# jiangzhengkai/mxdetection

Measured on AMD Instinct MI355X. Metric: images/sec (whole node) Faster R-CNN R50-FPN 3x800x1333, higher is better.
Workload: dtype bf16; 1 GPU; Faster R-CNN ResNet-50-FPN bf16 train step, batch 2/GPU, 3x800x1333 (padded 1344); global_batch=2, parallelism=dp1, frozen=stem+C2, frozen BN folded, optimizer=SGD momentum 0.9 wd 1e-4, launch=hipGraph replay, input=resident, wgrad_side_stream=True, rpn_branch_stream=True, grouped_wgrad=True, filter_prefetch_hints=True, params_trainable=41538304

## Files before the change

include/mxdet.h:

```cpp
#ifndef MXDET_H_
#define MXDET_H_

#include <stddef.h>
#include <stdint.h>

#ifdef __cplusplus
extern "C" {
#endif

#define MXDET_OK 0
#define MXDET_EINVAL (-1)
#define MXDET_ESHAPE (-2)
#define MXDET_EWORKSPACE (-3)
#define MXDET_EHIP (-4)
#define MXDET_ERCCL (-5)

#define MXDET_DTYPE_F32 0
#define MXDET_DTYPE_BF16 1

typedef void* mxdet_stream_t;

const char* mxdet_last_error(void);
const char* mxdet_version(void);

// ... 355 lines not shown
  float eps;
  int32_t relu;
  int32_t accumulate;
} mxdet_gn_desc_t;
size_t mxdet_group_norm_workspace_bytes(const mxdet_gn_desc_t* d, int32_t backward);
int mxdet_group_norm_fwd(const mxdet_gn_desc_t* d, const uint16_t* x, const float* gamma, const float* beta, uint16_t* y,
                         float* mean, float* rstd, void* workspace, size_t workspace_bytes, mxdet_stream_t stream);
int mxdet_group_norm_bwd(const mxdet_gn_desc_t* d, const uint16_t* x, const uint16_t* dy, const uint16_t* y,
                         const float* mean, const float* rstd, const float* gamma, const float* beta, uint16_t* dx,
                         float* dgamma, float* dbeta, void* workspace, size_t workspace_bytes, mxdet_stream_t stream);

int mxdet_stem_conv7x7(const void* image, int32_t dtype, int32_t N, int32_t H, int32_t W,
                       const uint16_t* w, const float* bias, uint16_t* y, mxdet_stream_t stream);
int mxdet_stem_conv7x7_pool(const void* image, int32_t dtype, int32_t N, int32_t H, int32_t W,
                            const uint16_t* w, const float* bias, uint16_t* y, mxdet_stream_t stream);
int mxdet_maxpool3x3s2(const uint16_t* x, int32_t N, int32_t H, int32_t W, int32_t C, uint16_t* y,
                       mxdet_stream_t stream);
int mxdet_subsample2(const uint16_t* x, int32_t N, int32_t H, int32_t W, int32_t C, uint16_t* y,
                     mxdet_stream_t stream);
int mxdet_subsample2_bwd(const uint16_t* dy, int32_t N, int32_t H, int32_t W, int32_t C,
                         int32_t accumulate, uint16_t* dx, mxdet_stream_t stream);
int mxdet_upsample2_bwd(const uint16_t* dfine, int32_t N, int32_t Hf, int32_t Wf, int32_t C,
                        int32_t accumulate, uint16_t* dcoarse, mxdet_stream_t stream);
size_t mxdet_retina_detect_workspace_bytes(const mxdet_pyramid_t* p, int32_t N, int32_t pre_nms_top_n);
int mxdet_retina_detect(const mxdet_pyramid_t* p, int32_t N, const float* im_info, int32_t pre_nms_top_n,
                        float score_thresh, float nms_thresh, int32_t max_per_image, float* dets, int32_t* num_dets,
                        void* workspace, size_t workspace_bytes, mxdet_stream_t stream);
int mxdet_retina_detect_soft(const mxdet_pyramid_t* p, int32_t N, const float* im_info, int32_t pre_nms_top_n,
                             float score_thresh, float nms_thresh, int32_t max_per_image, float* dets,
                             int32_t* num_dets, void* workspace, size_t workspace_bytes, int32_t method, float sigma,
// ... 57 lines not shown
```

include/mxdet_debug.h:

```cpp
#ifndef MXDET_DEBUG_H_
#define MXDET_DEBUG_H_

#include <stdint.h>

#include "mxdet.h"

#ifdef __cplusplus
extern "C" {
#endif

int mxdet_debug_force_conv_cfg(int32_t cfg);
int mxdet_debug_force_wgrad_ksplit(int32_t ksplit);
int mxdet_debug_preprocess_direct(int32_t on);

#define MXDET_TUNE_T64 0
#define MXDET_TUNE_T128 1
#define MXDET_TUNE_PAR64 2
#define MXDET_TUNE_WG_TARGET 3
#define MXDET_TUNE_WG_MINSTEPS 4
#define MXDET_TUNE_WG_MAXSTEPS 5
#define MXDET_TUNE_T3_ENABLE 6
#define MXDET_TUNE_T3_TARGET 7
#define MXDET_TUNE_T3_MINSTEPS 8
#define MXDET_TUNE_T3_NS 9
#define MXDET_TUNE_TAIL 10
#define MXDET_TUNE_WG_NS 11
#define MXDET_TUNE_ROI_TABLE 12
#define MXDET_TUNE_ROI_ROWS 13
#define MXDET_TUNE_STATIC_TAPS 14
#define MXDET_TUNE_T128W 15
#define MXDET_TUNE_T3_MIX 16
#define MXDET_TUNE_SPLITK_TILE 17
#define MXDET_TUNE_T3_PER_ITEM 18
#define MXDET_TUNE_COUNT 19
int mxdet_debug_set_tuning(int32_t which, int64_t value);
int64_t mxdet_debug_get_tuning(int32_t which);


#define MXDET_ROUTE_CONV 1
#define MXDET_ROUTE_WGRAD 2
#define MXDET_ROUTE_CONV_GROUPED 3
#define MXDET_ROUTE_WGRAD_GROUPED 4
#define MXDET_ROUTE_RETINA_LOSS 5
#define MXDET_ROUTE_RETINA_LOSS_IOU 6
#define MXDET_ROUTE_RETINA_LOSS_QUALITY 7
#define MXDET_ROUTE_RETINA_LOSS_DFL 8
#define MXDET_ROUTE_WORDS 16
#define MXDET_ROUTE_MAX 4
int mxdet_debug_route_probe(int32_t on);
int mxdet_debug_route_read(int32_t* records, int32_t max_records);

// ... 9 lines not shown
```

mxdetection_amd/_lib.py:

```python
import ctypes as C
import os

_HERE = os.path.dirname(os.path.abspath(__file__))
LIB_PATH = os.environ.get("MXDET_LIB") or os.path.join(_HERE, "libmxdet_hip.so")

c_i32, c_i64, c_u32, c_f32, c_sz, c_vp = C.c_int32, C.c_int64, C.c_uint32, C.c_float, C.c_size_t, C.c_void_p


class PyramidT(C.Structure):
    _fields_ = [
        ("num_levels", c_i32), ("A", c_i32),
        ("H", c_i32 * 8), ("W", c_i32 * 8), ("stride", c_i32 * 8),
        ("cls", c_vp * 8), ("reg", c_vp * 8),
        ("cls_sn", c_i64 * 8), ("cls_sy", c_i64 * 8), ("cls_sx", c_i64 * 8), ("cls_sa", c_i64 * 8),
        ("reg_sn", c_i64 * 8), ("reg_sy", c_i64 * 8), ("reg_sx", c_i64 * 8), ("reg_sc", c_i64 * 8),
        ("dtype", c_i32), ("classes", c_i32),
        ("base_anchors", c_vp * 8),
    ]


class FeatPyramidT(C.Structure):
    _fields_ = [
        ("num_levels", c_i32), ("lvl_min", c_i32),
        ("H", c_i32 * 8), ("W", c_i32 * 8),
# ... 187 lines not shown
    "mxdet_deform_im2col": (c_i32, [P(DeformDescT), c_vp, c_vp, c_vp, c_vp]),
    "mxdet_deform_col2im_coord": (c_i32, [P(DeformDescT), c_vp, c_vp, c_vp, c_vp, c_vp]),
    "mxdet_deform_col2im_workspace_bytes": (c_sz, [P(DeformDescT)]),
    "mxdet_deform_col2im": (c_i32, [P(DeformDescT), c_vp, c_vp, c_vp, c_vp, c_sz, c_vp]),
    "mxdet_dpool_fwd": (c_i32, [P(DpoolDescT), c_vp, c_vp, c_i64, c_vp, c_vp, c_vp, c_vp]),
    "mxdet_dpool_bwd_trans": (c_i32, [P(DpoolDescT), c_vp, c_vp, c_i64, c_vp, c_vp, c_vp, c_vp, c_vp, c_vp]),
    "mxdet_dpool_bwd_feat_workspace_bytes": (c_sz, [P(DpoolDescT), c_i64]),
    "mxdet_dpool_bwd_feat": (c_i32, [P(DpoolDescT), c_vp, c_vp, c_i64, c_vp, c_vp, c_vp, c_vp, c_sz, c_vp]),
    "mxdet_group_norm_workspace_bytes": (c_sz, [P(GnDescT), c_i32]),
    "mxdet_group_norm_fwd": (c_i32, [P(GnDescT), c_vp, c_vp, c_vp, c_vp, c_vp, c_vp, c_vp, c_sz, c_vp]),
    "mxdet_group_norm_bwd": (c_i32, [P(GnDescT), c_vp, c_vp, c_vp, c_vp, c_vp, c_vp, c_vp, c_vp, c_vp, c_vp, c_vp, c_sz,
                                     c_vp]),
    "mxdet_debug_group_norm_route": (c_i32, [P(GnDescT)]),
    "mxdet_stem_conv7x7": (c_i32, [c_vp, c_i32, c_i32, c_i32, c_i32, c_vp, c_vp, c_vp, c_vp]),
    "mxdet_stem_conv7x7_pool": (c_i32, [c_vp, c_i32, c_i32, c_i32, c_i32, c_vp, c_vp, c_vp, c_vp]),
    "mxdet_maxpool3x3s2": (c_i32, [c_vp, c_i32, c_i32, c_i32, c_i32, c_vp, c_vp]),
    "mxdet_subsample2": (c_i32, [c_vp, c_i32, c_i32, c_i32, c_i32, c_vp, c_vp]),
    "mxdet_subsample2_bwd": (c_i32, [c_vp, c_i32, c_i32, c_i32, c_i32, c_i32, c_vp, c_vp]),
    "mxdet_upsample2_bwd": (c_i32, [c_vp, c_i32, c_i32, c_i32, c_i32, c_i32, c_vp, c_vp]),
    "mxdet_add_bf16": (c_i32, [c_vp, c_vp, c_i64, c_vp, c_vp]),
    "mxdet_relu_bwd_bf16": (c_i32, [c_vp, c_vp, c_i64, c_vp, c_vp]),
    "mxdet_f32_to_bf16": (c_i32, [c_vp, c_i64, c_vp, c_vp]),
    "mxdet_f32_accum_to_bf16": (c_i32, [c_vp, c_i64, c_i32, c_vp, c_vp]),
    "mxdet_nchw_to_nhwc_bf16": (c_i32, [c_vp, c_i32, c_i32, c_i32, c_i32, c_i32, c_vp, c_vp]),
    "mxdet_nhwc_to_nchw_f32": (c_i32, [c_vp, c_i32, c_i32, c_i32, c_i32, c_vp, c_vp]),
    "mxdet_sgd_momentum_update": (c_i32, [c_vp, c_vp, c_vp, c_vp, c_i64, c_f32, c_f32, c_f32, c_f32, c_vp]),
    "mxdet_sgd_momentum_update_sched": (c_i32, [c_vp, c_vp, c_vp, c_vp, c_i64, c_vp, c_f32, c_f32, c_f32, c_vp]),
    "mxdet_comm_unique_id": (c_i32, [c_vp]),
    "mxdet_comm_create": (c_i32, [c_vp, c_i32, c_i32, P(c_vp)]),
    "mxdet_comm_destroy": (c_i32, [c_vp]),
    "mxdet_allreduce_bucket": (c_i32, [c_vp, c_vp, c_i64, c_vp, P(c_i32)]),
    "mxdet_comm_wait": (c_i32, [c_vp, c_i32, c_vp]),
    "mxdet_comm_broadcast": (c_i32, [c_vp, c_vp, c_sz, c_i32, c_vp]),
    "mxdet_debug_set_tuning": (c_i32, [c_i32, c_i64]),
    "mxdet_debug_get_tuning": (c_i64, [c_i32]),
    "mxdet_debug_route_probe": (c_i32, [c_i32]),
    "mxdet_debug_route_read": (c_i32, [P(c_i32), c_i32]),
}

DEBUG_SYMBOLS = ("mxdet_debug_force_conv_cfg", "mxdet_debug_force_wgrad_ksplit", "mxdet_debug_preprocess_direct",
                 "mxdet_debug_set_tuning", "mxdet_debug_get_tuning", "mxdet_debug_route_probe", "mxdet_debug_route_read",
                 "mxdet_debug_group_norm_route")
TUNING_KEYS = {"T64": 0, "T128": 1, "PAR64": 2, "WG_TARGET": 3, "WG_MINSTEPS": 4, "WG_MAXSTEPS": 5, "T3_ENABLE": 6,
               "T3_TARGET": 7, "T3_MINSTEPS": 8, "T3_NS": 9, "TAIL": 10, "WG_NS": 11, "ROI_TABLE": 12, "ROI_ROWS": 13, "STATIC_TAPS": 14,
               "T128W": 15, "T3_MIX": 16, "SPLITK_TILE": 17, "T3_PER_ITEM": 18}
ROUTE_KINDS = {"CONV": 1, "WGRAD": 2, "CONV_GROUPED": 3, "WGRAD_GROUPED": 4, "RETINA_LOSS": 5, "RETINA_LOSS_IOU": 6,
               "RETINA_LOSS_QUALITY": 7, "RETINA_LOSS_DFL": 8}

IOU_LOSS_KINDS = {"iou": 0, "giou": 1, "diou": 2}
CLS_LOSS_KINDS = {"qfl": 1, "vfl": 2}
CLS_LOSS_KINDS_DFL = {"focal": 0, "qfl": 1, "vfl": 2}
REG_MAX_LIMIT = 31

_lib = None


class MxdetError(RuntimeError):
    pass


# ... 38 lines not shown
```

mxdetection_amd/csrc/capi.hip:

```cpp
#include <stdarg.h>

#include "common.h"

namespace mxdet {

static thread_local char g_err[512] = {0};

void set_error(const char* fmt, ...) {
  va_list ap;
  va_start(ap, fmt);
  vsnprintf(g_err, sizeof(g_err), fmt, ap);
  va_end(ap);
}
void clear_error() { g_err[0] = 0; }

thread_local int g_route_probe = 0;
static thread_local int g_route_n = 0;
static thread_local int32_t g_route[kRouteMax][kRouteWords];
void route_record(const int32_t (&rec)[kRouteWords]) {
  if (g_route_n < kRouteMax) memcpy(g_route[g_route_n], rec, sizeof(rec));
  ++g_route_n;
}

static const long long kTuneDefault[MXDET_TUNE_COUNT] = {400, 1536, 1600, 3072, 64, 128, 1, 1536, 32, 2, 2, 2, 0, 2, 1, 1000000, 1, 0, 192};
static long long g_tune[MXDET_TUNE_COUNT] = {400, 1536, 1600, 3072, 64, 128, 1, 1536, 32, 2, 2, 2, 0, 2, 1, 1000000, 1, 0, 192};
long long tuning(int which) { return g_tune[which]; }

}

extern "C" const char* mxdet_last_error(void) { return mxdet::g_err; }
extern "C" const char* mxdet_version(void) { return "mxdet-hip 0.2 gfx950"; }

extern "C" int mxdet_debug_set_tuning(int32_t which, int64_t value) {
  mxdet::clear_error();
  MXDET_REQUIRE(which >= 0 && which < MXDET_TUNE_COUNT, MXDET_EINVAL, "debug_set_tuning: unknown key %d", which);
  mxdet::g_tune[which] = value < 0 ? mxdet::kTuneDefault[which] : (long long)value;
  return MXDET_OK;
}

extern "C" int64_t mxdet_debug_get_tuning(int32_t which) {
// ... 20 lines not shown
```

mxdetection_amd/csrc/dense_misc.hip:

```cpp
#include "common.h"

namespace mxdet {

typedef __attribute__((ext_vector_type(8))) short s16x8_t;

constexpr int STEM_PW = 264;
constexpr int STEM_PLANE = 7 * STEM_PW;
constexpr int STEM_K = 160;

__global__ void __launch_bounds__(256)
stem_conv_kernel(const void* __restrict__ img, int dtype, int N, int H, int W, int Ho, int Wo,
                 const uint16_t* __restrict__ w, const float* __restrict__ bias,
                 uint16_t* __restrict__ y) {
  constexpr int PATCH_ELEMS = (3 * STEM_PLANE + 8 + 7) & ~7;
  constexpr int MAIN_BYTES = (PATCH_ELEMS + 64 * STEM_K) * 2;
  constexpr int EP_BYTES = 4 * 32 * 68 * 4;
  __shared__ __attribute__((aligned(16))) unsigned char smem_raw[MAIN_BYTES > EP_BYTES ? MAIN_BYTES : EP_BYTES];
  __shared__ int koff[STEM_K];
  uint16_t* patch = (uint16_t*)smem_raw;
  uint16_t* wl = patch + PATCH_ELEMS;
  float* ep = (float*)smem_raw;
  const int tid = threadIdx.x, lane = tid & 63, wid = tid >> 6;
  const int wtiles = ceil_div(Wo, 128);
  int b = blockIdx.x;
// ... 94 lines not shown
constexpr int SP_PW = 296;
constexpr int SP_ROWS = 15;
constexpr int SP_PATCH_BYTES = SP_ROWS * SP_PW * 8;
constexpr int SP_HB_BYTES = 2 * 128 * 64 * 2;
constexpr int SP_LDS = SP_PATCH_BYTES > SP_HB_BYTES ? SP_PATCH_BYTES : SP_HB_BYTES;

template <typename T>
__device__ __forceinline__ float stem_px(const T* p);
template <>
__device__ __forceinline__ float stem_px<float>(const float* p) { return *p; }
template <>
__device__ __forceinline__ float stem_px<uint16_t>(const uint16_t* p) { return bf16_bits_to_f32(*p); }

template <typename T>
__global__ void __launch_bounds__(256, 2)
stem_pool_kernel(const T* __restrict__ img, int N, int H, int W, int Ho, int Wo, int Hp, int Wp,
                 const uint16_t* __restrict__ w, const float* __restrict__ bias, uint16_t* __restrict__ y) {
  __shared__ __attribute__((aligned(16))) unsigned char smem[SP_LDS];
  const int tid = threadIdx.x, lane = tid & 63;
  const int wid = __builtin_amdgcn_readfirstlane(tid >> 6);
  const int wm = wid >> 1, wn = wid & 1;
  const int frow = lane & 15, fq = lane >> 4;
  const int wtiles = ceil_div(Wp, SP_PC), htiles = ceil_div(Hp, 2);
  int b = blockIdx.x;
  const int wt = b % wtiles; b /= wtiles;
  const int ht = b % htiles;
  const int n = b / htiles;
  const int ph0 = 2 * ht, pw0 = wt * SP_PC;
  const int cr0 = 2 * ph0 - 1, cc0 = 2 * pw0 - 1;
  const int ir0 = 2 * cr0 - 3, ic0 = 2 * cc0 - 3;

  {
// ... 128 lines not shown
    if (ph >= Hp || pwg >= Wp) continue;
    const uint4 a = *(const uint4*)(hb + (q * 128 + 2 * pw) * 64 + cg * 8);
    const uint4 c = *(const uint4*)(hb + (q * 128 + 2 * pw + 1) * 64 + cg * 8);
    const uint4 d = *(const uint4*)(hb + (q * 128 + 2 * pw + 2) * 64 + cg * 8);
    auto mx = [](unsigned x, unsigned y2) {
      const unsigned lo = (x & 0xffffu) > (y2 & 0xffffu) ? (x & 0xffffu) : (y2 & 0xffffu);
      const unsigned hi = (x >> 16) > (y2 >> 16) ? (x >> 16) : (y2 >> 16);
      return lo | (hi << 16);
    };
    uint4 o;
    o.x = mx(mx(a.x, c.x), d.x); o.y = mx(mx(a.y, c.y), d.y); o.z = mx(mx(a.z, c.z), d.z); o.w = mx(mx(a.w, c.w), d.w);
    *(uint4*)(y + (((size_t)n * Hp + ph) * Wp + pwg) * 64 + cg * 8) = o;
  }
}


__global__ void maxpool3x3s2_kernel(const uint16_t* __restrict__ x, int N, int H, int W, int C, int Ho,
                                    int Wo, uint16_t* __restrict__ y) {
  const int CG = C >> 3;
  long long idx = (long long)blockIdx.x * blockDim.x + threadIdx.x;
  long long total = (long long)N * Ho * Wo * CG;
  if (idx >= total) return;
  int cg = (int)(idx % CG);
  long long pix = idx / CG;
  int wo = (int)(pix % Wo);
  long long t = pix / Wo;
  int ho = (int)(t % Ho), n = (int)(t / Ho);
  float m[8];
#pragma unroll
  for (int k = 0; k < 8; ++k) m[k] = -3.0e38f;
// ... 216 lines not shown
                     N, H, W, Ho, Wo, w, bias, y);
  return check_launch("stem_conv7x7");
}

extern "C" int mxdet_stem_conv7x7_pool(const void* image, int32_t dtype, int32_t N, int32_t H, int32_t W,
                                       const uint16_t* w, const float* bias, uint16_t* y, mxdet_stream_t stream) {
  clear_error();
  MXDET_REQUIRE(N > 0 && H > 0 && W > 0, MXDET_ESHAPE, "stem_conv7x7_pool: bad shape");
  MXDET_REQUIRE(dtype == MXDET_DTYPE_F32 || dtype == MXDET_DTYPE_BF16, MXDET_EINVAL, "stem_conv7x7_pool: dtype");
  MXDET_REQUIRE(image && w && y, MXDET_EINVAL, "stem_conv7x7_pool: null pointer");
  const int Ho = (H + 6 - 7) / 2 + 1, Wo = (W + 6 - 7) / 2 + 1;
  const int Hp = (Ho + 2 - 3) / 2 + 1, Wp = (Wo + 2 - 3) / 2 + 1;
  const long long nwg = (long long)N * ceil_div(Hp, 2) * ceil_div(Wp, SP_PC);
  MXDET_REQUIRE(nwg < (1ll << 31), MXDET_ESHAPE, "stem_conv7x7_pool: image too large");
  if (dtype == MXDET_DTYPE_F32)
    hipLaunchKernelGGL(stem_pool_kernel<float>, dim3((unsigned)nwg), dim3(256), 0, as_stream(stream), (const float*)image,
                       N, H, W, Ho, Wo, Hp, Wp, w, bias, y);
  else
    hipLaunchKernelGGL(stem_pool_kernel<uint16_t>, dim3((unsigned)nwg), dim3(256), 0, as_stream(stream),
                       (const uint16_t*)image, N, H, W, Ho, Wo, Hp, Wp, w, bias, y);
  return check_launch("stem_conv7x7_pool");
}

extern "C" int mxdet_maxpool3x3s2(const uint16_t* x, int32_t N, int32_t H, int32_t W, int32_t C,
                                  uint16_t* y, mxdet_stream_t stream) {
  clear_error();
  MXDET_REQUIRE(N > 0 && H > 0 && W > 0 && C > 0 && C % 8 == 0, MXDET_ESHAPE, "maxpool3x3s2: bad shape");
  MXDET_REQUIRE(x && y, MXDET_EINVAL, "maxpool3x3s2: null pointer");
  int Ho = (H + 2 - 3) / 2 + 1, Wo = (W + 2 - 3) / 2 + 1;
  long long total = (long long)N * Ho * Wo * (C / 8);
  hipLaunchKernelGGL(maxpool3x3s2_kernel, dim3(blocks_for(total, 256)), dim3(256), 0, as_stream(stream), x,
                     N, H, W, C, Ho, Wo, y);
  return check_launch("maxpool3x3s2");
}

extern "C" int mxdet_subsample2(const uint16_t* x, int32_t N, int32_t H, int32_t W, int32_t C,
// ... 124 lines not shown
```

mxdetection_amd/models/backbones/resnet.py:

```python
import os

import torch

from ...ops import dense
from ..utils.layers import ConvLayer, DeformConvLayer, cached_buf


BITMASKS = os.environ.get("MXDET_TUNE_RELU_BITS", "1") == "1"
CHAIN_FROZEN = os.environ.get("MXDET_TUNE_CHAIN", "1") != "0"
CHAIN3_FROZEN = os.environ.get("MXDET_TUNE_CHAIN", "2") not in ("0", "1")


class Bottleneck:
    def __init__(self, name, cin, planes, stride, downsample, trainable, need_dx, arena, ws, device, gen, dcn=None):
        kw = dict(arena=arena, ws=ws, device=device, gen=gen, trainable=trainable, train_bias=False)
        self.trainable, self.need_dx = trainable, need_dx
        self.conv3 = ConvLayer(name + ".conv3", planes, planes * 4, 1, init_std=0.25 * (2.0 / planes) ** 0.5, **kw)
        self.dcn = dcn is not None
        if self.dcn:
            assert trainable, "deformable convolutions only in trainable stages"
            self.conv2 = DeformConvLayer(name + ".conv2", planes, planes, stride, dcn["groups"], dcn["modulated"],
                                         arena=arena, ws=ws, device=device, gen=gen)
        else:
            self.conv2 = ConvLayer(name + ".conv2", planes, planes, 3, stride, **kw)
# ... 104 lines not shown
        cins = [64, 256, 512, 1024]
        for si in (3, 2, 1, 0):
            planes = 64 << si
            trainable = si > frozen_stages - 1 and si >= 1 if frozen_stages >= 1 else True
            stage = []
            for bi in reversed(range(blocks[si])):
                cin = cins[si] if bi == 0 else planes * 4
                stride = 2 if (bi == 0 and si > 0) else 1
                need_dx = trainable and not (bi == 0 and (si == 0 or si - 1 < frozen_stages))
                stage.insert(0, Bottleneck("layer%d.%d" % (si + 1, bi), cin, planes, stride, bi == 0, trainable,
                                           need_dx, arena, ws, device, gen,
                                           dcn=dcn if si + 2 in dcn_stages else None))
            self.stages[si] = stage
        self.stem_w = (torch.randn((64, 7, 7, 3), generator=gen) * (2.0 / 147) ** 0.5).to(torch.bfloat16).to(device)
        self.stem_b = torch.zeros((64,), dtype=torch.float32, device=device)
        self.bufs = {}
        self.outs = None
        self.front_override = None
        self.eager_parity = 0
        self.front_outs = []

    def layers(self):
        return [l for st in self.stages for b in st for l in b.layers()]

    def plan(self, image_shape):
        N, _, H, W = image_shape
        s = (N, ((H - 1) // 2 + 1 - 1) // 2 + 1, ((W - 1) // 2 + 1 - 1) // 2 + 1, 64)
        shapes = []
        for st in self.stages:
            for b in st:
# ... 2 lines not shown
        return shapes

    def forward(self, image):
        if self.front_override is not None:
            return self.forward_rest(self.front_override)
        return self.forward_rest(self.forward_front(image, self.eager_parity))

    def frozen_front(self):
        n = 0
        for st in self.stages:
            if any(b.trainable for b in st):
                break
            n += 1
        return n

    def forward_front(self, image, parity=0):
        N, _, H, W = image.shape
        H1, W1 = (H - 1) // 2 + 1, (W - 1) // 2 + 1
        dev = self.stem_w.device
        x = dense.stem_conv7x7_pool(image, self.stem_w, self.stem_b,
                                    cached_buf(self.bufs, "pool", (N, (H1 - 1) // 2 + 1, (W1 - 1) // 2 + 1, 64),
                                               torch.bfloat16, dev))
        nf = self.frozen_front()
        if nf > 0:
            self.stages[nf - 1][-1].y_key = "y%d" % parity if parity else "y"
        self.front_outs = []
        for st in self.stages[:nf]:
            x = self._stage_forward(st, x, None)
            self.front_outs.append(x)
        return x

    def _stage_forward(self, st, x, xb):
        ready = False
        for i, b in enumerate(st):
            nb = st[i + 1] if i + 1 < len(st) else None
            ride = (CHAIN3_FROZEN and nb is not None and b.chainable() and nb.chainable() and nb.down is None and
                    nb.conv1.cout == 64 and nb.conv1.stride == 1)
# ... 37 lines not shown
```

mxdetection_amd/models/utils/checkpoint.py:

```python
import torch


class CheckpointMixin:
    def export_params(self):
        out = {"stem.weight": self.backbone.stem_w.float().cpu(), "stem.bias": self.backbone.stem_b.float().cpu()}
        frozen = [l for st in self.backbone.stages for b in st for l in b.layers() if not l.trainable]
        for l in self.layers + frozen:
            out[l.name + ".weight"] = l.w_bf16.float().cpu()
            if l.has_bias:
                out[l.name + ".bias"] = l.bias_f32.float().cpu()
        for l in getattr(self, "norm_layers", ()):
            for name, idx in l.named_params():
                out[name] = self.arena.view(idx, "w").float().cpu()
        return out


    def _named_tensors(self):
        out = [("stem.weight", "frozen", self.backbone.stem_w, None), ("stem.bias", "frozen", self.backbone.stem_b, None)]
        frozen = [l for st in self.backbone.stages for b in st for l in b.layers() if not l.trainable]
        seen = set()
        for l in list(self.layers) + frozen:
            if id(l) in seen:
                continue
            seen.add(id(l))
# ... 71 lines not shown
            by_name[name] = layer
            a = blob.get("arg:" + name)
            if a is None:
                missing.append(name)
                continue
            t.copy_(self._from_mx(a, t, layer).to(t.dtype))
        for i, e in enumerate(self.arena.entries):
            a = blob.get("aux:momentum:" + e[0])
            if a is not None:
                m = self.arena.view(i, "m")
                m.copy_(self._from_mx(a, m, by_name.get(e[0])))
        if strict and missing:
            raise KeyError("checkpoint lacks %d parameters, e.g. %s" % (len(missing), missing[:3]))
        self.arena.refresh_bf16()
        self.refresh_transposed()
        return missing

    def export_grads(self):
        return {e[0]: self.arena.view(i, "g").float().cpu() for i, e in enumerate(self.arena.entries)}

    def num_params(self):
        return sum(e[3] for e in self.arena.entries)
```

mxdetection_amd/models/utils/detector.py:

```python
import contextlib
import os

import torch

from ...utils.hipgraph import GraphEvent
from .checkpoint import CheckpointMixin
from .dp import BucketReducer, make_comm
from .layers import ParamArena, Workspace
from .schedule import CapturedStep, ReplayScratch, ScheduleRecorder, begin_capture, uncovered_ranges


_PROBE_STREAMS = []
_ABL = frozenset(t for t in os.environ.get("MXDET_ABL_SKIP", "").split(",") if t)
Workspace.abl_skip = _ABL


class DetectorBase(CheckpointMixin):
    def _init_base(self, device):
        self.device = device
        self.arena = ParamArena(device)
        self.ws = Workspace(device)
        self.planned = None
        self.dist = None
        self.comm = None
# ... 168 lines not shown
    @contextlib.contextmanager
    def _weights_restored(self):
        snap = (self.arena.w.clone(), self.arena.m.clone())
        yield
        torch.cuda.synchronize()
        self.arena.w.copy_(snap[0])
        self.arena.m.copy_(snap[1])
        self.arena.refresh_bf16()
        self.refresh_transposed()
        del snap
        torch.cuda.synchronize()

    def capture(self, image, gt_boxes, im_info, lr, image_offset=0, warmup=2, gt_masks=None, momentum=0.9, wd=1e-4):
        dev = self.device
        hyper = (float(momentum), float(wd))
        self.static_in = (image.clone(), gt_boxes.clone(), im_info.clone())
        self.static_masks = gt_masks.clone() if gt_masks is not None else None
        self.step_dev = torch.zeros((1,), dtype=torch.int32, device=dev)
        self.lr_dev = torch.full((1,), float(lr), dtype=torch.float32, device=dev)
        self._lr_host = lr

        def eager_step(step):
            self.train_step(*self.static_in, step=step, image_offset=image_offset, lr=lr, gt_masks=self.static_masks,
                            momentum=hyper[0], wd=hyper[1])
        if warmup > 0:
            with self._weights_restored():
                for i in range(warmup):
                    eager_step(i)
        torch.cuda.synchronize()
        cap = CapturedStep()
# ... 178 lines not shown
```

mxdetection_amd/ops/dense.py:

```python
import ctypes as C

import torch

from .. import _lib
from .._lib import ConvDescT, check, ptr, stream_ptr

_DT = {torch.float32: 0, torch.bfloat16: 1}


def mem_range(*tensors):
    spans = [(t.data_ptr(), t.numel() * t.element_size()) for t in tensors]
    bases = {t.untyped_storage().data_ptr() for t in tensors}
    if len(bases) == 1:
        lo = min(p for p, _ in spans)
        hi = max(p + n for p, n in spans)
        if hi - lo <= 2 * sum(n for _, n in set(spans)):
            return (lo, hi - lo)
    return spans[0]


def conv_desc(N, H, W, Cin, Cout, KH, KW, stride, pad, relu=False, res_upsample=False, accumulate=False, prefetch=None,
              relu_bits=None):
    d = ConvDescT()
    if relu_bits is not None:
# ... 224 lines not shown
    check(_lib.load().mxdet_filter_transpose_batched(ptr(table), ndesc, total_tiles, stream_ptr()),
          "filter_transpose_batched")


def stem_conv7x7(image, w, bias=None, out=None):
    lib = _lib.load()
    N, _, H, W = image.shape
    Ho, Wo = (H - 1) // 2 + 1, (W - 1) // 2 + 1
    if out is None:
        out = torch.empty((N, Ho, Wo, 64), dtype=torch.bfloat16, device=image.device)
    check(lib.mxdet_stem_conv7x7(ptr(image), _DT[image.dtype], N, H, W, ptr(w), ptr(bias), ptr(out), stream_ptr()),
          "stem_conv7x7")
    return out


def stem_conv7x7_pool(image, w, bias=None, out=None):
    lib = _lib.load()
    N, _, H, W = image.shape
    Ho, Wo = (H - 1) // 2 + 1, (W - 1) // 2 + 1
    Hp, Wp = (Ho - 1) // 2 + 1, (Wo - 1) // 2 + 1
    if out is None:
        out = torch.empty((N, Hp, Wp, 64), dtype=torch.bfloat16, device=image.device)
    check(lib.mxdet_stem_conv7x7_pool(ptr(image), _DT[image.dtype], N, H, W, ptr(w), ptr(bias), ptr(out), stream_ptr()),
          "stem_conv7x7_pool")
    return out


def maxpool3x3s2(x, out=None):
    lib = _lib.load()
    N, H, W, Cc = x.shape
    Ho, Wo = (H - 1) // 2 + 1, (W - 1) // 2 + 1
    if out is None:
        out = torch.empty((N, Ho, Wo, Cc), dtype=torch.bfloat16, device=x.device)
    check(lib.mxdet_maxpool3x3s2(ptr(x), N, H, W, Cc, ptr(out), stream_ptr()), "maxpool3x3s2")
    return out


# ... 107 lines not shown
```

mxdetection_amd/utils/pretrained.py:

```python
import numpy as np

from .params_io import fold_batchnorm, load_params

_BLOCKS = {50: (3, 4, 6, 3), 101: (3, 4, 23, 3)}


def resnet_v1_names(depth):
    yield "stem", "conv0_weight", "bn0"
    for si, nb in enumerate(_BLOCKS[depth]):
        for bi in range(nb):
            u, ours = "stage%d_unit%d" % (si + 1, bi + 1), "layer%d.%d" % (si + 1, bi)
            for k in (1, 2, 3):
                yield "%s.conv%d" % (ours, k), "%s_conv%d_weight" % (u, k), "%s_bn%d" % (u, k)
            if bi == 0:
                yield ours + ".down", u + "_sc_weight", u + "_sc_bn"


def _get(blob, name):
    for k in ("arg:" + name, "aux:" + name, name):
        if k in blob:
            return np.asarray(blob[k])
    return None


# ... 13 lines not shown
            continue
        wf, bf = fold_batchnorm(w, stats[0], stats[1], stats[2], stats[3], eps=eps, fix_gamma=fix_gamma)
        tw, tb = tensors[ours + ".weight"], tensors[ours + ".bias"]
        src = torch.from_numpy(wf).permute(0, 2, 3, 1).contiguous()
        khwc = getattr(layers[ours + ".weight"], "dcn_khwc", None)
        if khwc is not None and tuple(src.shape[1:]) == tuple(khwc):
            src = src.reshape(tw.shape)
        if tuple(src.shape) != tuple(tw.shape):
            raise ValueError("%s: %s has shape %s, the model expects %s" % (ours, wname, tuple(src.shape), tuple(tw.shape)))
        tw.copy_(src.to(tw.device).to(tw.dtype))
        tb.copy_(torch.from_numpy(bf).to(tb.device).to(tb.dtype))
    if strict and missing:
        raise KeyError("pretrained file lacks %d backbone tensors, e.g. %s" % (len(missing), missing[:3]))
    model.arena.refresh_bf16()
    model.refresh_transposed()
    return missing
```

Measured before the change: 476.3 images/sec.

## Stream stem conv+pool through a row ring buffer with prepacked MFMA filter fragments

Adds a new fused stem 7x7 conv + 3x3 maxpool kernel. Each workgroup walks several pooled row pairs over a column strip, keeping a 16-row image ring in LDS and prefetching the next rows into registers while the MFMAs run, so overlapping input rows are reused instead of reloaded per tile. The stem filter is repacked once into MFMA fragment layout outside the captured graph, and each wave loads it straight into registers. The new route is on by default through a tuning knob. It needs extra state to keep the prepared filter in sync with weight updates, but the stem is frozen here, so this should hold.

```diff
diff --git a/include/mxdet.h b/include/mxdet.h
--- a/include/mxdet.h
+++ b/include/mxdet.h
@@ -393,6 +393,11 @@
                        const uint16_t* w, const float* bias, uint16_t* y, mxdet_stream_t stream);
 int mxdet_stem_conv7x7_pool(const void* image, int32_t dtype, int32_t N, int32_t H, int32_t W,
                             const uint16_t* w, const float* bias, uint16_t* y, mxdet_stream_t stream);
+#define MXDET_STEM_FRAG_BYTES 28672
+int mxdet_stem_filter_prepare(const uint16_t* w, uint16_t* frag, mxdet_stream_t stream);
+int mxdet_stem_conv7x7_pool_prepared(const void* image, int32_t dtype, int32_t N, int32_t H, int32_t W,
+                                     const uint16_t* w, const uint16_t* frag, const float* bias, uint16_t* y,
+                                     mxdet_stream_t stream);
 int mxdet_maxpool3x3s2(const uint16_t* x, int32_t N, int32_t H, int32_t W, int32_t C, uint16_t* y,
                        mxdet_stream_t stream);
 int mxdet_subsample2(const uint16_t* x, int32_t N, int32_t H, int32_t W, int32_t C, uint16_t* y,
diff --git a/include/mxdet_debug.h b/include/mxdet_debug.h
--- a/include/mxdet_debug.h
+++ b/include/mxdet_debug.h
@@ -32,9 +32,11 @@
 #define MXDET_TUNE_T3_MIX 16
 #define MXDET_TUNE_SPLITK_TILE 17
 #define MXDET_TUNE_T3_PER_ITEM 18
-#define MXDET_TUNE_COUNT 19
+#define MXDET_TUNE_STEM_STREAM 19
+#define MXDET_TUNE_COUNT 20
 int mxdet_debug_set_tuning(int32_t which, int64_t value);
 int64_t mxdet_debug_get_tuning(int32_t which);
+int mxdet_debug_stem_stream_geometry(int32_t* strip, int32_t* run_pairs);
 
 
 #define MXDET_ROUTE_CONV 1
diff --git a/mxdetection_amd/_lib.py b/mxdetection_amd/_lib.py
--- a/mxdetection_amd/_lib.py
+++ b/mxdetection_amd/_lib.py
@@ -225,6 +225,9 @@
     "mxdet_debug_group_norm_route": (c_i32, [P(GnDescT)]),
     "mxdet_stem_conv7x7": (c_i32, [c_vp, c_i32, c_i32, c_i32, c_i32, c_vp, c_vp, c_vp, c_vp]),
     "mxdet_stem_conv7x7_pool": (c_i32, [c_vp, c_i32, c_i32, c_i32, c_i32, c_vp, c_vp, c_vp, c_vp]),
+    "mxdet_stem_filter_prepare": (c_i32, [c_vp, c_vp, c_vp]),
+    "mxdet_stem_conv7x7_pool_prepared": (c_i32, [c_vp, c_i32, c_i32, c_i32, c_i32, c_vp, c_vp, c_vp, c_vp, c_vp]),
+    "mxdet_debug_stem_stream_geometry": (c_i32, [P(c_i32), P(c_i32)]),
     "mxdet_maxpool3x3s2": (c_i32, [c_vp, c_i32, c_i32, c_i32, c_i32, c_vp, c_vp]),
     "mxdet_subsample2": (c_i32, [c_vp, c_i32, c_i32, c_i32, c_i32, c_vp, c_vp]),
     "mxdet_subsample2_bwd": (c_i32, [c_vp, c_i32, c_i32, c_i32, c_i32, c_i32, c_vp, c_vp]),
@@ -251,10 +254,10 @@
 
 DEBUG_SYMBOLS = ("mxdet_debug_force_conv_cfg", "mxdet_debug_force_wgrad_ksplit", "mxdet_debug_preprocess_direct",
                  "mxdet_debug_set_tuning", "mxdet_debug_get_tuning", "mxdet_debug_route_probe", "mxdet_debug_route_read",
-                 "mxdet_debug_group_norm_route")
+                 "mxdet_debug_group_norm_route", "mxdet_debug_stem_stream_geometry")
 TUNING_KEYS = {"T64": 0, "T128": 1, "PAR64": 2, "WG_TARGET": 3, "WG_MINSTEPS": 4, "WG_MAXSTEPS": 5, "T3_ENABLE": 6,
                "T3_TARGET": 7, "T3_MINSTEPS": 8, "T3_NS": 9, "TAIL": 10, "WG_NS": 11, "ROI_TABLE": 12, "ROI_ROWS": 13, "STATIC_TAPS": 14,
-               "T128W": 15, "T3_MIX": 16, "SPLITK_TILE": 17, "T3_PER_ITEM": 18}
+               "T128W": 15, "T3_MIX": 16, "SPLITK_TILE": 17, "T3_PER_ITEM": 18, "STEM_STREAM": 19}
 ROUTE_KINDS = {"CONV": 1, "WGRAD": 2, "CONV_GROUPED": 3, "WGRAD_GROUPED": 4, "RETINA_LOSS": 5, "RETINA_LOSS_IOU": 6,
                "RETINA_LOSS_QUALITY": 7, "RETINA_LOSS_DFL": 8}
 
diff --git a/mxdetection_amd/csrc/capi.hip b/mxdetection_amd/csrc/capi.hip
--- a/mxdetection_amd/csrc/capi.hip
+++ b/mxdetection_amd/csrc/capi.hip
@@ -22,8 +22,8 @@
   ++g_route_n;
 }
 
-static const long long kTuneDefault[MXDET_TUNE_COUNT] = {400, 1536, 1600, 3072, 64, 128, 1, 1536, 32, 2, 2, 2, 0, 2, 1, 1000000, 1, 0, 192};
-static long long g_tune[MXDET_TUNE_COUNT] = {400, 1536, 1600, 3072, 64, 128, 1, 1536, 32, 2, 2, 2, 0, 2, 1, 1000000, 1, 0, 192};
+static const long long kTuneDefault[MXDET_TUNE_COUNT] = {400, 1536, 1600, 3072, 64, 128, 1, 1536, 32, 2, 2, 2, 0, 2, 1, 1000000, 1, 0, 192, 1};
+static long long g_tune[MXDET_TUNE_COUNT] = {400, 1536, 1600, 3072, 64, 128, 1, 1536, 32, 2, 2, 2, 0, 2, 1, 1000000, 1, 0, 192, 1};
 long long tuning(int which) { return g_tune[which]; }
 
 }
diff --git a/mxdetection_amd/csrc/dense_misc.hip b/mxdetection_amd/csrc/dense_misc.hip
--- a/mxdetection_amd/csrc/dense_misc.hip
+++ b/mxdetection_amd/csrc/dense_misc.hip
@@ -132,8 +132,8 @@
 
 template <typename T>
 __global__ void __launch_bounds__(256, 2)
-stem_pool_kernel(const T* __restrict__ img, int N, int H, int W, int Ho, int Wo, int Hp, int Wp,
-                 const uint16_t* __restrict__ w, const float* __restrict__ bias, uint16_t* __restrict__ y) {
+stem_pool_oneshot_kernel(const T* __restrict__ img, int N, int H, int W, int Ho, int Wo, int Hp, int Wp,
+                         const uint16_t* __restrict__ w, const float* __restrict__ bias, uint16_t* __restrict__ y) {
   __shared__ __attribute__((aligned(16))) unsigned char smem[SP_LDS];
   const int tid = threadIdx.x, lane = tid & 63;
   const int wid = __builtin_amdgcn_readfirstlane(tid >> 6);
@@ -292,6 +292,223 @@
   }
 }
 
+constexpr int SS_MT = 2;
+constexpr int SS_MG = 1;
+constexpr int SS_R = 2;
+constexpr int SS_COLS = 32 * SS_MT;
+constexpr int SS_PC = SS_MT == 2 ? 28 : 56;
+constexpr int SS_LC = 2 * SS_COLS;
+constexpr int SS_PW = SS_LC + 8;
+constexpr int SS_RPP = 256 / SS_LC;
+constexpr int SS_NPASS = 8 / SS_RPP;
+constexpr int SS_RING_BYTES = 16 * SS_PW * 8;
+constexpr int SS_HB_BYTES = 2 * SS_COLS * 64 * 2;
+static_assert(SS_MT == 2 || SS_MT == 4, "strip geometry");
+static_assert(2 * SS_PC + 1 <= SS_COLS && 2 * (2 * SS_PC) + 7 <= SS_LC, "the strip's stem columns and their patch are covered");
+
+__global__ void stem_filter_frag_kernel(const uint16_t* __restrict__ w, uint16_t* __restrict__ frag) {
+  const int idx = blockIdx.x * blockDim.x + threadIdx.x;
+  if (idx >= 2 * 2 * 7 * 64) return;
+  const int lane = idx & 63, kh = (idx >> 6) % 7, nj = (idx >> 6) / 7;
+  const int frow = lane & 15, fq = lane >> 4;
+  const uint16_t* wr = w + (nj * 16 + frow) * 147;
+  s16x8_t v;
+#pragma unroll
+  for (int e = 0; e < 8; ++e) {
+    const int kw = 2 * fq + (e >> 2), c = e & 3;
+    v[e] = (kw < 7 && c < 3) ? (short)wr[(kh * 7 + kw) * 3 + c] : (short)0;
+  }
+  *(s16x8_t*)(frag + (size_t)idx * 8) = v;
+}
+
+template <typename T>
+__device__ __forceinline__ float stem_raw(T v);
+template <>
+__device__ __forceinline__ float stem_raw<float>(float v) { return v; }
+template <>
+__device__ __forceinline__ float stem_raw<uint16_t>(uint16_t v) { return bf16_bits_to_f32(v); }
+
+template <typename T>
+__global__ void __launch_bounds__(256, 4)
+stem_pool_kernel(const T* __restrict__ img, int N, int H, int W, int Ho, int Wo, int Hp, int Wp,
+                 const uint16_t* __restrict__ frag, const float* __restrict__ bias, uint16_t* __restrict__ y) {
+  __shared__ __attribute__((aligned(16))) unsigned char smem[SS_RING_BYTES + SS_HB_BYTES];
+  unsigned char* ring = smem;
+  uint16_t* hb = (uint16_t*)(smem + SS_RING_BYTES);
+  const int tid = threadIdx.x, lane = tid & 63;
+  const int wid = __builtin_amdgcn_readfirstlane(tid >> 6);
+  const int wm = wid >> 1, wn = wid & 1;
+  const int frow = lane & 15, fq = lane >> 4;
+  const int wtiles = ceil_div(Wp, SS_PC), pairs = ceil_div(Hp, 2), runs = ceil_div(pairs, SS_R);
+  int b = blockIdx.x;
+  const int wt = b % wtiles; b /= wtiles;
+  const int run = b % runs;
+  const int n = b / runs;
+  const int pair0 = run * SS_R;
+  const int nt = (pairs - pair0) < SS_R ? (pairs - pair0) : SS_R;
+  const int ph0 = 2 * pair0, pw0 = wt * SS_PC;
+  const int cr0 = 2 * ph0 - 1, cc0 = 2 * pw0 - 1;
+  const int ir0 = 2 * cr0 - 3, ic0 = 2 * cc0 - 3;
+
+  bf16x8_t bw[2][7];
+  {
+    const bf16x8_t* fr = (const bf16x8_t*)frag + (size_t)(wn * 2) * 7 * 64 + lane;
+#pragma unroll
+    for (int j = 0; j < 2; ++j)
+#pragma unroll
+      for (int kh = 0; kh < 7; ++kh) bw[j][kh] = fr[(j * 7 + kh) * 64];
+  }
+  float bz[2];
+#pragma unroll
+  for (int j = 0; j < 2; ++j) bz[j] = bias ? bias[wn * 32 + j * 16 + frow] : 0.0f;
+
+  if (tid < 16 * 8) *(uint2*)(ring + ((size_t)(tid >> 3) * SS_PW + SS_LC + (tid & 7)) * 8) = make_uint2(0u, 0u);
+
+  const int lcol = tid % SS_LC, lrow = tid / SS_LC;
+  const int wi = ic0 + lcol;
+  const bool cok = wi >= 0 && wi < W;
+  const unsigned plane = (unsigned)H * W;
+  const char* base = (const char*)(img + (size_t)(n * 3) * plane);
+  const unsigned wic = (unsigned)(wi < 0 ? 0 : (wi >= W ? W - 1 : wi));
+  auto issue = [&](T (&raw)[SS_NPASS][3], int r0) {
+#pragma unroll
+    for (int p = 0; p < SS_NPASS; ++p) {
+      const int hi = ir0 + r0 + p * SS_RPP + lrow;
+      const unsigned off = ((unsigned)(hi < 0 ? 0 : (hi >= H ? H - 1 : hi)) * (unsigned)W + wic) * (unsigned)sizeof(T);
+      raw[p][0] = *(const T*)(base + off);
+      raw[p][1] = *(const T*)(base + (off + plane * (unsigned)sizeof(T)));
+      raw[p][2] = *(const T*)(base + (off + 2 * plane * (unsigned)sizeof(T)));
+    }
+  };
+  auto commit = [&](const T (&raw)[SS_NPASS][3], int r0) {
+#pragma unroll
+    for (int p = 0; p < SS_NPASS; ++p) {
+      const int r = r0 + p * SS_RPP + lrow;
+      const int hi = ir0 + r;
+      const bool ok = cok && hi >= 0 && hi < H;
+      uint2 o;
+      o.x = (unsigned)f32_to_bf16_bits(stem_raw<T>(raw[p][0])) | ((unsigned)f32_to_bf16_bits(stem_raw<T>(raw[p][1])) << 16);
+      o.y = (unsigned)f32_to_bf16_bits(stem_raw<T>(raw[p][2]));
+      if (!ok) o = make_uint2(0u, 0u);
+      if (r >= 0) *(uint2*)(ring + ((size_t)(r & 15) * SS_PW + lcol) * 8) = o;
+    }
+  };
+  T raw[SS_NPASS][3];
+  {
+    T raw0[SS_NPASS][3];
+    issue(raw0, -1);
+    issue(raw, 7);
+    commit(raw0, -1);
+    commit(raw, 7);
+  }
+  __syncthreads();
+
+  typedef __attribute__((ext_vector_type(2))) unsigned short u16x2_t;
+  typedef __attribute__((ext_vector_type(2))) __bf16 bf16x2_t;
+  u16x2_t pmax[2][SS_MT][2][2];
+#pragma unroll
+  for (int q = 0; q < 2; ++q)
+#pragma unroll
+    for (int i = 0; i < SS_MT; ++i)
+#pragma unroll
+      for (int j = 0; j < 2; ++j)
+#pragma unroll
+        for (int r = 0; r < 2; ++r) pmax[q][i][j][r] = (u16x2_t){0, 0};
+  auto put_hb = [&](int q) {
+#pragma unroll
+    for (int i = 0; i < SS_MT; ++i)
+#pragma unroll
+      for (int j = 0; j < 2; ++j)
+#pragma unroll
+        for (int r = 0; r < 4; ++r)
+          hb[(q * SS_COLS + wm * (16 * SS_MT) + i * 16 + fq * 4 + r) * 64 + wn * 32 + j * 16 + frow] =
+              q == 0 ? pmax[0][i][j][r >> 1][r & 1] : pmax[1][i][j][r >> 1][r & 1];
+  };
+  const bool interior = cr0 >= 0 && cr0 + 4 * nt + 1 <= Ho && cc0 >= 0 && cc0 + SS_COLS <= Wo;
+#pragma unroll 1
+  for (int t = 0; t < nt; ++t) {
+    const bool more = t + 1 < nt;
+    if (more) issue(raw, 8 * t + 15);
+#pragma unroll 1
+    for (int js = (t == 0 ? 0 : 1); js < 5; ++js) {
+      const int rb = 8 * t + 2 * js;
+      const int crow = cr0 + 4 * t + js;
+      const bool rowok = crow >= 0 && crow < Ho;
+#pragma unroll
+      for (int i0 = 0; i0 < SS_MT; i0 += SS_MG) {
+        f32x4_t acc[SS_MG][2];
+#pragma unroll
+        for (int i = 0; i < SS_MG; ++i)
+#pragma unroll
+          for (int j = 0; j < 2; ++j) acc[i][j] = (f32x4_t){0.f, 0.f, 0.f, 0.f};
+#pragma unroll
+        for (int kh = 0; kh < 7; ++kh) {
+          bf16x8_t af[SS_MG];
+          const unsigned char* rowp = ring + (size_t)((rb + kh) & 15) * (SS_PW * 8);
+#pragma unroll
+          for (int i = 0; i < SS_MG; ++i) {
+            const int col = wm * (16 * SS_MT) + (i0 + i) * 16 + frow;
+            af[i] = *(const bf16x8_t*)(rowp + (size_t)(2 * col + 2 * fq) * 8);
+          }
+#pragma unroll
+          for (int i = 0; i < SS_MG; ++i)
+#pragma unroll
+            for (int j = 0; j < 2; ++j)
+              acc[i][j] = __builtin_amdgcn_mfma_f32_16x16x32_bf16(af[i], bw[j][kh], acc[i][j], 0, 0, 0);
+        }
+#pragma unroll
+        for (int i = 0; i < SS_MG; ++i) {
+          const int ccb = cc0 + wm * (16 * SS_MT) + (i0 + i) * 16 + fq * 4;
+#pragma unroll
+          for (int j = 0; j < 2; ++j) {
+            float v[4];
+#pragma unroll
+            for (int r = 0; r < 4; ++r) {
+              v[r] = fmaxf(acc[i][j][r] + bz[j], 0.0f);
+              if (!interior) v[r] = (rowok && ccb + r >= 0 && ccb + r < Wo) ? v[r] : 0.0f;
+            }
+#pragma unroll
+            for (int h = 0; h < 2; ++h) {
+              const bf16x2_t pk = (bf16x2_t){(__bf16)v[2 * h], (__bf16)v[2 * h + 1]};
+              const u16x2_t u = __builtin_bit_cast(u16x2_t, pk);
+              if (js >= 2) pmax[1][i0 + i][j][h] = __builtin_elementwise_max(pmax[1][i0 + i][j][h], u);
+              if (js <= 2) pmax[0][i0 + i][j][h] = __builtin_elementwise_max(pmax[0][i0 + i][j][h], u);
+              if (js == 4) pmax[0][i0 + i][j][h] = u;
+            }
+          }
+        }
+      }
+      if (js == 2) put_hb(0);
+    }
+    put_hb(1);
+#pragma unroll
+    for (int i = 0; i < SS_MT; ++i)
+#pragma unroll
+      for (int j = 0; j < 2; ++j)
+#pragma unroll
+        for (int r = 0; r < 2; ++r) pmax[1][i][j][r] = (u16x2_t){0, 0};
+    __syncthreads();
+    if (more) commit(raw, 8 * t + 15);
+    for (int it = tid; it < 2 * SS_PC * 8; it += 256) {
+      const int cg = it & 7, pw = (it >> 3) % SS_PC, q = (it >> 3) / SS_PC;
+      const int ph = ph0 + 2 * t + q, pwg = pw0 + pw;
+      if (ph >= Hp || pwg >= Wp) continue;
+      const uint4 a = *(const uint4*)(hb + (q * SS_COLS + 2 * pw) * 64 + cg * 8);
+      const uint4 c = *(const uint4*)(hb + (q * SS_COLS + 2 * pw + 1) * 64 + cg * 8);
+      const uint4 d = *(const uint4*)(hb + (q * SS_COLS + 2 * pw + 2) * 64 + cg * 8);
+      auto mx = [](unsigned x, unsigned y2) {
+        const unsigned lo = (x & 0xffffu) > (y2 & 0xffffu) ? (x & 0xffffu) : (y2 & 0xffffu);
+        const unsigned hi = (x >> 16) > (y2 >> 16) ? (x >> 16) : (y2 >> 16);
+        return lo | (hi << 16);
+      };
+      uint4 o;
+      o.x = mx(mx(a.x, c.x), d.x); o.y = mx(mx(a.y, c.y), d.y); o.z = mx(mx(a.z, c.z), d.z); o.w = mx(mx(a.w, c.w), d.w);
+      *(uint4*)(y + (((size_t)n * Hp + ph) * Wp + pwg) * 64 + cg * 8) = o;
+    }
+    __syncthreads();
+  }
+}
+
 
 __global__ void maxpool3x3s2_kernel(const uint16_t* __restrict__ x, int N, int H, int W, int C, int Ho,
                                     int Wo, uint16_t* __restrict__ y) {
@@ -538,12 +755,50 @@
   const long long nwg = (long long)N * ceil_div(Hp, 2) * ceil_div(Wp, SP_PC);
   MXDET_REQUIRE(nwg < (1ll << 31), MXDET_ESHAPE, "stem_conv7x7_pool: image too large");
   if (dtype == MXDET_DTYPE_F32)
+    hipLaunchKernelGGL(stem_pool_oneshot_kernel<float>, dim3((unsigned)nwg), dim3(256), 0, as_stream(stream),
+                       (const float*)image, N, H, W, Ho, Wo, Hp, Wp, w, bias, y);
+  else
+    hipLaunchKernelGGL(stem_pool_oneshot_kernel<uint16_t>, dim3((unsigned)nwg), dim3(256), 0, as_stream(stream),
+                       (const uint16_t*)image, N, H, W, Ho, Wo, Hp, Wp, w, bias, y);
+  return check_launch("stem_conv7x7_pool");
+}
+
+extern "C" int mxdet_stem_filter_prepare(const uint16_t* w, uint16_t* frag, mxdet_stream_t stream) {
+  clear_error();
+  MXDET_REQUIRE(w && frag, MXDET_EINVAL, "stem_filter_prepare: null pointer");
+  MXDET_REQUIRE(((uintptr_t)frag & 15) == 0, MXDET_EINVAL, "stem_filter_prepare: frag must be 16-byte aligned");
+  hipLaunchKernelGGL(stem_filter_frag_kernel, dim3(MXDET_STEM_FRAG_BYTES / 16 / 256), dim3(256), 0, as_stream(stream), w, frag);
+  return check_launch("stem_filter_prepare");
+}
+
+extern "C" int mxdet_stem_conv7x7_pool_prepared(const void* image, int32_t dtype, int32_t N, int32_t H, int32_t W,
+                                                const uint16_t* w, const uint16_t* frag, const float* bias, uint16_t* y,
+                                                mxdet_stream_t stream) {
+  if (tuning(MXDET_TUNE_STEM_STREAM) == 0) return mxdet_stem_conv7x7_pool(image, dtype, N, H, W, w, bias, y, stream);
+  clear_error();
+  MXDET_REQUIRE(N > 0 && H > 0 && W > 0, MXDET_ESHAPE, "stem_conv7x7_pool_prepared: bad shape");
+  MXDET_REQUIRE(dtype == MXDET_DTYPE_F32 || dtype == MXDET_DTYPE_BF16, MXDET_EINVAL, "stem_conv7x7_pool_prepared: dtype");
+  MXDET_REQUIRE(image && frag && y, MXDET_EINVAL, "stem_conv7x7_pool_prepared: null pointer");
+  MXDET_REQUIRE(((uintptr_t)frag & 15) == 0, MXDET_EINVAL, "stem_conv7x7_pool_prepared: frag must be 16-byte aligned");
+  const int Ho = (H + 6 - 7) / 2 + 1, Wo = (W + 6 - 7) / 2 + 1;
+  const int Hp = (Ho + 2 - 3) / 2 + 1, Wp = (Wo + 2 - 3) / 2 + 1;
+  const long long nwg = (long long)N * ceil_div(ceil_div(Hp, 2), SS_R) * ceil_div(Wp, SS_PC);
+  MXDET_REQUIRE(nwg < (1ll << 31) && 3ll * H * W < (1ll << 30), MXDET_ESHAPE, "stem_conv7x7_pool_prepared: image too large");
+  if (dtype == MXDET_DTYPE_F32)
     hipLaunchKernelGGL(stem_pool_kernel<float>, dim3((unsigned)nwg), dim3(256), 0, as_stream(stream), (const float*)image,
-                       N, H, W, Ho, Wo, Hp, Wp, w, bias, y);
+                       N, H, W, Ho, Wo, Hp, Wp, frag, bias, y);
   else
     hipLaunchKernelGGL(stem_pool_kernel<uint16_t>, dim3((unsigned)nwg), dim3(256), 0, as_stream(stream),
-                       (const uint16_t*)image, N, H, W, Ho, Wo, Hp, Wp, w, bias, y);
-  return check_launch("stem_conv7x7_pool");
+                       (const uint16_t*)image, N, H, W, Ho, Wo, Hp, Wp, frag, bias, y);
+  return check_launch("stem_conv7x7_pool_prepared");
+}
+
+extern "C" int mxdet_debug_stem_stream_geometry(int32_t* strip, int32_t* run_pairs) {
+  clear_error();
+  MXDET_REQUIRE(strip && run_pairs, MXDET_EINVAL, "debug_stem_stream_geometry: null pointer");
+  *strip = SS_PC;
+  *run_pairs = SS_R;
+  return MXDET_OK;
 }
 
 extern "C" int mxdet_maxpool3x3s2(const uint16_t* x, int32_t N, int32_t H, int32_t W, int32_t C,
diff --git a/mxdetection_amd/models/backbones/resnet.py b/mxdetection_amd/models/backbones/resnet.py
--- a/mxdetection_amd/models/backbones/resnet.py
+++ b/mxdetection_amd/models/backbones/resnet.py
@@ -142,6 +142,9 @@
             self.stages[si] = stage
         self.stem_w = (torch.randn((64, 7, 7, 3), generator=gen) * (2.0 / 147) ** 0.5).to(torch.bfloat16).to(device)
         self.stem_b = torch.zeros((64,), dtype=torch.float32, device=device)
+        self._stem_frag = None
+        self._stem_frag_key = None
+        self.stem_frag()
         self.bufs = {}
         self.outs = None
         self.front_override = None
@@ -174,13 +177,27 @@
             n += 1
         return n
 
+    def stem_frag(self):
+        if not dense.stem_stream_route():
+            return None
+        w = self.stem_w
+        key = self._stem_frag_key
+        if key is not None and key[0] is w and key[1] == w._version:
+            return self._stem_frag
+        if torch.cuda.is_current_stream_capturing():
+            raise RuntimeError("stem_w changed since its prepared image was built: call backbone.stem_frag() before "
+                               "capturing (the prepare launch does not belong in a step's graph)")
+        self._stem_frag = dense.stem_filter_prepare(w, self._stem_frag)
+        self._stem_frag_key = (w, w._version)
+        return self._stem_frag
+
     def forward_front(self, image, parity=0):
         N, _, H, W = image.shape
         H1, W1 = (H - 1) // 2 + 1, (W - 1) // 2 + 1
         dev = self.stem_w.device
         x = dense.stem_conv7x7_pool(image, self.stem_w, self.stem_b,
                                     cached_buf(self.bufs, "pool", (N, (H1 - 1) // 2 + 1, (W1 - 1) // 2 + 1, 64),
-                                               torch.bfloat16, dev))
+                                               torch.bfloat16, dev), frag=self.stem_frag())
         nf = self.frozen_front()
         if nf > 0:
             self.stages[nf - 1][-1].y_key = "y%d" % parity if parity else "y"
diff --git a/mxdetection_amd/models/utils/checkpoint.py b/mxdetection_amd/models/utils/checkpoint.py
--- a/mxdetection_amd/models/utils/checkpoint.py
+++ b/mxdetection_amd/models/utils/checkpoint.py
@@ -109,6 +109,7 @@
             raise KeyError("checkpoint lacks %d parameters, e.g. %s" % (len(missing), missing[:3]))
         self.arena.refresh_bf16()
         self.refresh_transposed()
+        self.backbone.stem_frag()
         return missing
 
     def export_grads(self):
diff --git a/mxdetection_amd/models/utils/detector.py b/mxdetection_amd/models/utils/detector.py
--- a/mxdetection_amd/models/utils/detector.py
+++ b/mxdetection_amd/models/utils/detector.py
@@ -206,6 +206,7 @@
     def capture(self, image, gt_boxes, im_info, lr, image_offset=0, warmup=2, gt_masks=None, momentum=0.9, wd=1e-4):
         dev = self.device
         hyper = (float(momentum), float(wd))
+        self.backbone.stem_frag()
         self.static_in = (image.clone(), gt_boxes.clone(), im_info.clone())
         self.static_masks = gt_masks.clone() if gt_masks is not None else None
         self.step_dev = torch.zeros((1,), dtype=torch.int32, device=dev)
diff --git a/mxdetection_amd/ops/dense.py b/mxdetection_amd/ops/dense.py
--- a/mxdetection_amd/ops/dense.py
+++ b/mxdetection_amd/ops/dense.py
@@ -262,13 +262,44 @@
     return out
 
 
-def stem_conv7x7_pool(image, w, bias=None, out=None):
+STEM_FRAG_ELEMS = 2 * 2 * 7 * 64 * 8
+
+
+def stem_stream_route():
+    lib = _lib.load()
+    if getattr(lib, "mxdet_stem_conv7x7_pool_prepared", None) is None:
+        return False
+    return lib.mxdet_debug_get_tuning(_lib.TUNING_KEYS["STEM_STREAM"]) == 1
+
+
+def stem_stream_geometry():
+    import ctypes as C
+    strip, run = C.c_int32(), C.c_int32()
+    check(_lib.load().mxdet_debug_stem_stream_geometry(C.byref(strip), C.byref(run)), "debug_stem_stream_geometry")
+    return strip.value, run.value
+
+
+def stem_filter_prepare(w, out=None):
+    assert w.dtype == torch.bfloat16 and tuple(w.shape) == (64, 7, 7, 3) and w.is_contiguous()
+    if out is None:
+        out = torch.empty((STEM_FRAG_ELEMS,), dtype=torch.bfloat16, device=w.device)
+    check(_lib.load().mxdet_stem_filter_prepare(ptr(w), ptr(out), stream_ptr()), "stem_filter_prepare")
+    return out
+
+
+def stem_conv7x7_pool(image, w, bias=None, out=None, frag=None):
     lib = _lib.load()
     N, _, H, W = image.shape
     Ho, Wo = (H - 1) // 2 + 1, (W - 1) // 2 + 1
     Hp, Wp = (Ho - 1) // 2 + 1, (Wo - 1) // 2 + 1
     if out is None:
         out = torch.empty((N, Hp, Wp, 64), dtype=torch.bfloat16, device=image.device)
+    if stem_stream_route():
+        if frag is None:
+            frag = stem_filter_prepare(w)
+        check(lib.mxdet_stem_conv7x7_pool_prepared(ptr(image), _DT[image.dtype], N, H, W, ptr(w), ptr(frag), ptr(bias),
+                                                   ptr(out), stream_ptr()), "stem_conv7x7_pool_prepared")
+        return out
     check(lib.mxdet_stem_conv7x7_pool(ptr(image), _DT[image.dtype], N, H, W, ptr(w), ptr(bias), ptr(out), stream_ptr()),
           "stem_conv7x7_pool")
     return out
diff --git a/mxdetection_amd/utils/pretrained.py b/mxdetection_amd/utils/pretrained.py
--- a/mxdetection_amd/utils/pretrained.py
+++ b/mxdetection_amd/utils/pretrained.py
@@ -51,4 +51,5 @@
         raise KeyError("pretrained file lacks %d backbone tensors, e.g. %s" % (len(missing), missing[:3]))
     model.arena.refresh_bf16()
     model.refresh_transposed()
+    model.backbone.stem_frag()
     return missing
```

Measured after the change: 476.3 images/sec. About the same (-0.0%).
